# mila-iqia/babyai

Hardware: AMD Instinct MI355X
Metric: env-steps/sec (higher is better)
Workload: dtype u8; 1 GPU; BabyAI-BossLevel-v0 56x56x3 pixel (RGBImgPartialObsWrapper) obs, 1048576 envs in total = 1048576 per GPU x 1, random actions, auto-reset; envs_per_gpu=1048576, total_envs=1048576, parallelism=env-shards x1, no collective

## Files before the change

babyai_amd/csrc/bbai_render.hpp:

```cpp
#pragma once
#include "bbai_types.hpp"

namespace bbai {

constexpr int RENDER_QUEUE_DEFAULT = 1;
constexpr int RENDER_QUEUE_PACED = 3;
constexpr int64_t RENDER_QUEUE_MIN_ENVS = 262144;

constexpr int CHUNKS_PER_ROW = PIX * 3 / 8;
constexpr int VEC_PER_ENV = PIX_BYTES / 16;

constexpr int LINE_BYTES = 128;
constexpr int DELTA_UNIT = 8;
constexpr int UNIT_LINES = DELTA_UNIT * PIX_BYTES / LINE_BYTES;
static_assert(DELTA_UNIT * PIX_BYTES % LINE_BYTES == 0 && PIX_BYTES % 64 == 0, "8-env units are whole 128-byte lines");
constexpr int RENDER_PIECE_DEFAULT = 64;

BB_HD uint64_t line_cells(int s, int t) {
    uint64_t m = 0;
    for (int b = s; b < t; b += 8) {
        const int ch = b >> 3, py = ch / CHUNKS_PER_ROW, cx = ch - py * CHUNKS_PER_ROW;
        m |= 1ull << ((cx / 3) * VIEW + (py >> 3));
    }
    return m;
}

BB_HD constexpr uint32_t chunk_half_recipe(int byte) {
    const int row = byte / (PIX * 3), xb = byte - row * (PIX * 3);
    const int cell = xb / (TILE * 3) * VIEW + row / TILE;
    const int off = row % TILE * (TILE * 3) + xb % (TILE * 3);
    return (uint32_t)cell | (uint32_t)off << 8;
}
BB_HD constexpr uint32_t chunk_recipe(int k) { return chunk_half_recipe(16 * k) | chunk_half_recipe(16 * k + 8) << 16; }

BB_HD constexpr bool chunk_recipes_match_render_chunk() {
    for (int k = 0; k < VEC_PER_ENV; ++k) {
        uint32_t w = 0;
        for (int h = 0; h < 2; ++h) {
            const int ch = 2 * k + h;
            const int py = ch / CHUNKS_PER_ROW, cx = ch - py * CHUNKS_PER_ROW;
            const int ti = cx / 3, part = cx - ti * 3;
            const int tj = py >> 3, ty = py & 7;
            const int cell = ti * VIEW + tj, off = ty * 24 + part * 8;
            if (cell < 0 || cell >= VIEW * VIEW || off < 0 || off + 8 > TILE_BYTES) return false;
            w |= ((uint32_t)cell | (uint32_t)off << 8) << (16 * h);
        }
        if (chunk_recipe(k) != w) return false;
    }
    return true;
}
static_assert(TILE == 8 && TILE_BYTES <= 256 && VIEW * VIEW <= 256, "a cell and a tile offset fit a byte each");
static_assert(chunk_recipes_match_render_chunk(), "chunk_recipe(k) = render_chunk's (cell, offset) of chunks 2k and 2k + 1, for every k");

template <int P>
struct Pieces {
    static_assert(P == 16 || P == 32 || P == 64, "pieces of 16, 32 or 64 bytes");
    static_assert(PIX_BYTES % P == 0, "whole pieces per env");
    static constexpr int NP = PIX_BYTES / P;
    static constexpr int S = P / 16;
};

}

#if defined(__HIPCC__)
#include "bbai_kernels.hpp"

using namespace bbai;

__device__ __forceinline__ void load_atlas_lds(uint8_t* s_atlas, const uint8_t* atlas, int n_tiles, int tid, int T) {
    for (int k = tid; k < n_tiles * TILE_BYTES / 8; k += T) ((uint64_t*)s_atlas)[k] = ((const uint64_t*)atlas)[k];
}
__device__ __forceinline__ void load_lut_lds(uint8_t* s_lut, const uint8_t* lut, int tid, int T) {
    for (int k = tid; k < 512; k += T) s_lut[k] = lut[k];
}

__device__ __forceinline__ uint8_t tile_id(const uint8_t* s_lut, int o0, int o1, int o2, int cell) {
    const int key = o0 | (o1 << 3) | (o2 << 6);
    return s_lut[(cell == AGENT_CELL ? 256 : 0) + key];
}

__device__ __forceinline__ uint64_t render_chunk(const uint8_t* s_atlas, const uint8_t* tiles49, int ch) {
    const int py = ch / CHUNKS_PER_ROW, cx = ch - py * CHUNKS_PER_ROW;
    const int ti = cx / 3, part = cx - ti * 3;
    const int tj = py >> 3, ty = py & 7;
    const int tile = tiles49[ti * VIEW + tj];
    return *(const uint64_t*)(s_atlas + tile * TILE_BYTES + ty * 24 + part * 8);
}

__device__ __forceinline__ void store_chunk16(const uint8_t* s_atlas, const uint8_t* t49, int k, u32x4* dst) {
    const uint64_t lo = render_chunk(s_atlas, t49, 2 * k);
    const uint64_t hi = render_chunk(s_atlas, t49, 2 * k + 1);
    u32x4 v = {(uint32_t)lo, (uint32_t)(lo >> 32), (uint32_t)hi, (uint32_t)(hi >> 32)};
    __builtin_nontemporal_store(v, dst);
}

__device__ __forceinline__ void init_chunk_table(uint32_t* s_ct, int tid, int T) {
    for (int k = tid; k < bbai::VEC_PER_ENV; k += T) s_ct[k] = bbai::chunk_recipe(k);
}
__device__ __forceinline__ void store_chunk16_t(const uint8_t* s_atlas, const uint32_t* s_ct, const uint8_t* t49, int k, u32x4* dst) {
    const uint32_t w = s_ct[k];
    const uint32_t ta = t49[w & 0xff], tb = t49[(w >> 16) & 0xff];
    const uint64_t lo = *(const uint64_t*)(s_atlas + ta * TILE_BYTES + ((w >> 8) & 0xff));
    const uint64_t hi = *(const uint64_t*)(s_atlas + tb * TILE_BYTES + (w >> 24));
    u32x4 v = {(uint32_t)lo, (uint32_t)(lo >> 32), (uint32_t)hi, (uint32_t)(hi >> 32)};
    __builtin_nontemporal_store(v, dst);
}

template <int RENDER_GROUP, int RENDER_BLOCK>
__global__ __launch_bounds__(RENDER_BLOCK) void k_render(int64_t n, const uint8_t* __restrict__ image,
                                                         uint8_t* __restrict__ pixels, const uint8_t* __restrict__ atlas,
                                                         const uint8_t* __restrict__ lut, int n_tiles,
                                                         uint8_t* __restrict__ shadow ) {
    __shared__ __attribute__((aligned(16))) uint8_t s_atlas[MAX_TILES * TILE_BYTES];
    __shared__ uint8_t s_lut[512];
    __shared__ uint8_t s_tile[RENDER_GROUP * VIEW * VIEW + 8];
    load_atlas_lds(s_atlas, atlas, n_tiles, threadIdx.x, RENDER_BLOCK);
    load_lut_lds(s_lut, lut, threadIdx.x, RENDER_BLOCK);
    const int64_t ngroups = (n + RENDER_GROUP - 1) / RENDER_GROUP;
    for (int64_t grp = blockIdx.x; grp < ngroups; grp += gridDim.x) {
        const int64_t env0 = grp * RENDER_GROUP;
        const int ne = (int)(n - env0 < RENDER_GROUP ? n - env0 : RENDER_GROUP);
        __syncthreads();
        for (int c = threadIdx.x; c < ne * VIEW * VIEW; c += RENDER_BLOCK) {
            const int e = c / (VIEW * VIEW), cell = c - e * (VIEW * VIEW);
            const uint8_t* o = image + (env0 + e) * OBS_BYTES + cell * 3;
            s_tile[c] = tile_id(s_lut, o[0], o[1], o[2], cell);
            if (shadow) shadow[env0 * (VIEW * VIEW) + c] = s_tile[c];
        }
        __syncthreads();
        u32x4* out = (u32x4*)(pixels + env0 * PIX_BYTES);
        for (int q = threadIdx.x; q < ne * VEC_PER_ENV; q += RENDER_BLOCK) {
            const int e = q / VEC_PER_ENV, k = q - e * VEC_PER_ENV;
            store_chunk16(s_atlas, s_tile + e * (VIEW * VIEW), k, out + q);
        }
    }
}

template <int RENDER_GROUP, int RENDER_BLOCK, int NC, int K>
__global__ __launch_bounds__(RENDER_BLOCK) void k_render_q(int64_t n, const uint8_t* __restrict__ image,
                                                           uint8_t* __restrict__ pixels, const uint8_t* __restrict__ atlas,
                                                           const uint8_t* __restrict__ lut, int n_tiles, unsigned int* __restrict__ counters,
                                                           int pace_x16 ,
                                                           uint8_t* __restrict__ shadow ) {
    __shared__ __attribute__((aligned(16))) uint8_t s_atlas[MAX_TILES * TILE_BYTES];
    __shared__ uint8_t s_lut[512];
    __shared__ uint8_t s_tile[2][RENDER_GROUP * VIEW * VIEW + 8];
    __shared__ unsigned int s_ticket[2];
    __shared__ unsigned long long s_origin;
    load_atlas_lds(s_atlas, atlas, n_tiles, threadIdx.x, RENDER_BLOCK);
    load_lut_lds(s_lut, lut, threadIdx.x, RENDER_BLOCK);
    const int64_t all_groups = (n + RENDER_GROUP - 1) / RENDER_GROUP;
    const int64_t n_super = (all_groups + K - 1) / K;
    const unsigned int cidx = blockIdx.x % NC;
    unsigned int* counter = counters + 64 * cidx;
    int buf = 0, tp = 0;
    if (threadIdx.x == 0) {
        const unsigned int t0 = atomicAdd(counter, 1u);
        s_ticket[0] = t0;
        s_origin = __builtin_amdgcn_s_memrealtime() * 160ull - ((unsigned long long)t0 * NC + cidx) * (unsigned long long)pace_x16;
    }
    __syncthreads();
    for (;;) {
        const int64_t sg = (int64_t)s_ticket[tp] * NC + cidx;
        if (sg >= n_super) break;
        if (pace_x16) {
            const unsigned long long due = s_origin + (unsigned long long)sg * (unsigned long long)pace_x16;
            while (__builtin_amdgcn_s_memrealtime() * 160ull < due) __builtin_amdgcn_s_sleep(1);
        }
#pragma unroll
        for (int kk = 0; kk < K; ++kk) {
            const int64_t grp = sg * K + kk;
            if (grp >= all_groups) break;
            const int64_t env0 = grp * RENDER_GROUP;
            const int ne = (int)(n - env0 < RENDER_GROUP ? n - env0 : RENDER_GROUP);
            for (int c = threadIdx.x; c < ne * VIEW * VIEW; c += RENDER_BLOCK) {
                const int e = c / (VIEW * VIEW), cell = c - e * (VIEW * VIEW);
                const uint8_t* o = image + (env0 + e) * OBS_BYTES + cell * 3;
                s_tile[buf][c] = tile_id(s_lut, o[0], o[1], o[2], cell);
                if (shadow) shadow[env0 * (VIEW * VIEW) + c] = s_tile[buf][c];
            }
            if (kk == 0 && threadIdx.x == 0) s_ticket[tp ^ 1] = atomicAdd(counter, 1u);
            __syncthreads();
            u32x4* out = (u32x4*)(pixels + env0 * PIX_BYTES);
            for (int q = threadIdx.x; q < ne * VEC_PER_ENV; q += RENDER_BLOCK) {
                const int e = q / VEC_PER_ENV, k = q - e * VEC_PER_ENV;
                store_chunk16(s_atlas, s_tile[buf] + e * (VIEW * VIEW), k, out + q);
            }
            buf ^= 1;
        }
        tp ^= 1;
    }
    if (threadIdx.x == 0) {
        unsigned int* departed = counters + 64 * NC;
        if (atomicAdd(departed, 1u) == gridDim.x - 1) {
            for (int c = 0; c <= NC; ++c) atomicExch(counters + 64 * c, 0u);
        }
    }
}


__device__ __forceinline__ uint64_t delta_cell(const uint8_t* s_lut, uint32_t o0, uint32_t o1, uint32_t o2, uint32_t old, bool live, int lane,
                                               uint8_t* t49, uint8_t* shadow_row) {
    const uint32_t id = live ? tile_id(s_lut, o0, o1, o2, lane) : 0;
    const bool d = live && id != old;
    const uint64_t m = __ballot(d);
    if (live) t49[lane] = (uint8_t)id;
    if (d) shadow_row[lane] = (uint8_t)id;
    return m;
}

__device__ __forceinline__ void init_line_table(uint8_t* s_lea, uint64_t* s_lma, uint64_t* s_lmb, int tid, int T) {
    for (int l = tid; l < UNIT_LINES; l += T) {
        const int b0 = l * LINE_BYTES, b1 = b0 + LINE_BYTES;
        const int ea = b0 / PIX_BYTES, eb = (b1 - 1) / PIX_BYTES;
        s_lea[l] = (uint8_t)ea;
        s_lma[l] = line_cells(b0 - ea * PIX_BYTES, (eb != ea ? (ea + 1) * PIX_BYTES : b1) - ea * PIX_BYTES);
        s_lmb[l] = eb != ea ? line_cells(0, b1 - eb * PIX_BYTES) : 0;
    }
}

__device__ __forceinline__ void list_dirty_lines(const uint64_t* dmask, const uint8_t* s_lea, const uint64_t* s_lma, const uint64_t* s_lmb,
                                                 uint16_t* list, unsigned int* nd, int nl, int tid, int T) {
    const int lane = tid & 63;
    for (int L0 = tid - lane; L0 < nl; L0 += T) {
        const int L = L0 + lane;
        bool d = false;
        if (L < nl) {
            const int u = L / UNIT_LINES, l = L - u * UNIT_LINES, ea = u * DELTA_UNIT + s_lea[l];
            d = ((dmask[ea] & s_lma[l]) | (s_lmb[l] ? dmask[ea + 1] & s_lmb[l] : 0)) != 0;
        }
        const uint64_t m = __ballot(d);
        if (!m) continue;
        unsigned int base = 0;
        if (lane == 0) base = atomicAdd(nd, (unsigned int)__builtin_popcountll(m));
        base = __shfl(base, 0);
        if (d) list[base + __builtin_popcountll(m & ((1ull << lane) - 1))] = (uint16_t)L;
    }
}

__device__ __forceinline__ void store_listed_lines(const uint16_t* list, int nd, const uint8_t* s_atlas, const uint8_t* tiles, u32x4* out, int nq,
                                                   int tid, int T) {
    for (int i = tid; i < nd * 8; i += T) {
        const int q = (int)list[i >> 3] * 8 + (i & 7);
        if (q >= nq) continue;
        const int e = q / VEC_PER_ENV, k = q - e * VEC_PER_ENV;
        store_chunk16(s_atlas, tiles + e * CELLS, k, out + q);
    }
}

__device__ __forceinline__ void wave_lds_sync() {
    __builtin_amdgcn_fence(__ATOMIC_RELEASE, "workgroup");
    __builtin_amdgcn_wave_barrier();
    __builtin_amdgcn_fence(__ATOMIC_ACQUIRE, "workgroup");
}

template <int P>
__device__ __forceinline__ void init_piece_cells(uint64_t* s_pm, int tid, int nthreads) {
    for (int p = tid; p < Pieces<P>::NP; p += nthreads) s_pm[p] = line_cells(p * P, p * P + P);
}

template <int P>
__device__ __forceinline__ void store_dirty_pieces(uint64_t m, const uint64_t* s_pm, uint16_t* wl, const uint8_t* s_atlas, const uint32_t* s_ct,
                                                   const uint8_t* t49, u32x4* out, int lane) {
    constexpr int NP = Pieces<P>::NP, S = Pieces<P>::S;
    int cnt = 0;
    for (int p0 = 0; p0 < NP; p0 += 64) {
        const int p = p0 + lane;
        const bool d = p < NP && (m & s_pm[p]) != 0;
        const uint64_t b = __ballot(d);
        if (d) wl[cnt + __builtin_popcountll(b & ((1ull << lane) - 1))] = (uint16_t)p;
        cnt += __builtin_popcountll(b);
    }
    wave_lds_sync();
    for (int i = lane; i < cnt * S; i += 64) {
        const int k = (int)wl[i / S] * S + (i & (S - 1));
        store_chunk16_t(s_atlas, s_ct, t49, k, out + k);
    }
    wave_lds_sync();
}

template <int G, int T, int SCHED, int P>
__global__ __launch_bounds__(T) void k_render_delta(int64_t n, const uint8_t* __restrict__ image, uint8_t* __restrict__ pixels,
                                                    uint8_t* __restrict__ shadow ,
                                                    const uint8_t* __restrict__ atlas, const uint8_t* __restrict__ lut, int n_tiles) {
    static_assert(G % DELTA_UNIT == 0 && T % 64 == 0 && G % (T / 64) == 0, "whole units per group, whole envs per wave");
    constexpr int W = T / 64, EPW = G / W, GL = G / DELTA_UNIT * UNIT_LINES;
    __shared__ __attribute__((aligned(16))) uint8_t s_atlas[MAX_TILES * TILE_BYTES];
    __shared__ uint8_t s_lut[512];
    const int lane = threadIdx.x & 63, wave = threadIdx.x >> 6;
    const int64_t ngroups = (n + G - 1) / G;
    int64_t g, gend, gstep;
    if (SCHED == 0) { g = blockIdx.x; gend = ngroups; gstep = gridDim.x; }
    else { const int64_t per = (ngroups + gridDim.x - 1) / gridDim.x; g = blockIdx.x * per; gend = g + per < ngroups ? g + per : ngroups; gstep = 1; }
    uint32_t o0[EPW], o1[EPW], o2[EPW], old[EPW];
    auto load = [&](int64_t grp) {
#pragma unroll
        for (int j = 0; j < EPW; ++j) {
            const int64_t env = grp * G + wave + j * W;
            o0[j] = o1[j] = o2[j] = old[j] = 0;
            if (grp < gend && lane < CELLS && env < n) {
                const uint8_t* o = image + env * OBS_BYTES + lane * 3;
                o0[j] = o[0]; o1[j] = o[1]; o2[j] = o[2];
                old[j] = shadow[env * CELLS + lane];
            }
        }
    };
    load_atlas_lds(s_atlas, atlas, n_tiles, threadIdx.x, T);
    load_lut_lds(s_lut, lut, threadIdx.x, T);
    if constexpr (P < LINE_BYTES) {
        __shared__ uint64_t s_pm[Pieces<P>::NP];
        __shared__ uint16_t s_wl[W][Pieces<P>::NP];
        __shared__ uint8_t s_tile1[G * CELLS + 8];
        __shared__ uint32_t s_ct[VEC_PER_ENV];
        init_piece_cells<P>(s_pm, threadIdx.x, T);
        init_chunk_table(s_ct, threadIdx.x, T);
        load(g);
        __syncthreads();
        for (; g < gend; g += gstep) {
            const int64_t env0 = g * G;
            const int ne = (int)(n - env0 < G ? n - env0 : G);
            uint64_t dm[EPW];
#pragma unroll
            for (int j = 0; j < EPW; ++j) {
                const int e = wave + j * W;
                const bool live = lane < CELLS && e < ne;
                const uint32_t id = live ? tile_id(s_lut, o0[j], o1[j], o2[j], lane) : 0;
                const bool d = live && id != old[j];
                dm[j] = __ballot(d);
                if (live) s_tile1[e * CELLS + lane] = (uint8_t)id;
                if (d) shadow[(env0 + e) * CELLS + lane] = (uint8_t)id;
            }
            load(g + gstep);
            wave_lds_sync();
#pragma unroll
            for (int j = 0; j < EPW; ++j) {
                const int e = wave + j * W;
                if (dm[j]) store_dirty_pieces<P>(dm[j], s_pm, s_wl[wave], s_atlas, s_ct, s_tile1 + e * CELLS, (u32x4*)(pixels + (env0 + e) * PIX_BYTES), lane);
            }
        }
        return;
    } else {
    __shared__ uint64_t s_lma[UNIT_LINES], s_lmb[UNIT_LINES];
    __shared__ uint8_t s_lea[UNIT_LINES];
    __shared__ uint64_t s_dmask[2][G];
    __shared__ uint8_t s_tile[2][G * CELLS + 8];
    __shared__ uint16_t s_list[2][GL];
    __shared__ unsigned int s_nd[2];
    init_line_table(s_lea, s_lma, s_lmb, threadIdx.x, T);
    load(g);
    __syncthreads();
    int buf = 0;
    for (; g < gend; g += gstep, buf ^= 1) {
        const int64_t env0 = g * G;
        const int ne = (int)(n - env0 < G ? n - env0 : G);
#pragma unroll
        for (int j = 0; j < EPW; ++j) {
            const int e = wave + j * W;
            const uint64_t m = delta_cell(s_lut, o0[j], o1[j], o2[j], old[j], lane < CELLS && e < ne, lane, s_tile[buf] + e * CELLS, shadow + (env0 + e) * CELLS);
            if (lane == 0) s_dmask[buf][e] = m;
        }
        if (threadIdx.x == 0) s_nd[buf] = 0;
        __syncthreads();
        const int nl = (int)(((int64_t)ne * PIX_BYTES + LINE_BYTES - 1) / LINE_BYTES);
        list_dirty_lines(s_dmask[buf], s_lea, s_lma, s_lmb, s_list[buf], &s_nd[buf], nl, threadIdx.x, T);
        __syncthreads();
        const int64_t gn = g + gstep;
        load(gn);
        store_listed_lines(s_list[buf], (int)s_nd[buf], s_atlas, s_tile[buf], (u32x4*)(pixels + env0 * PIX_BYTES), ne * VEC_PER_ENV, threadIdx.x, T);
    }
    }
}

constexpr int DSTORE_PIECES = 32 * CELLS / 8;
template <int G, int T, int P>
__global__ __launch_bounds__(T) void k_render_dstore(int64_t n, uint8_t* __restrict__ pixels, const uint8_t* __restrict__ shadow ,
                                                     const uint64_t* __restrict__ dmask , const uint8_t* __restrict__ atlas, int n_tiles) {
    static_assert(G == 32 && T >= DSTORE_PIECES && T >= G && T % 64 == 0, "one 8-byte shadow piece per thread and group");
    constexpr int GL = G / DELTA_UNIT * UNIT_LINES;
    __shared__ __attribute__((aligned(16))) uint8_t s_atlas[MAX_TILES * TILE_BYTES];
    __shared__ __attribute__((aligned(8))) uint8_t s_tile[2][G * CELLS + 8];
    load_atlas_lds(s_atlas, atlas, n_tiles, threadIdx.x, T);
    const int tid = threadIdx.x, lane = tid & 63;
    const int64_t ngroups = (n + G - 1) / G;
    const int64_t gstep = gridDim.x;
    int64_t g = blockIdx.x;
    auto load_mask = [&](int64_t grp) -> uint64_t {
        const int64_t env = grp * G + tid;
        return (tid < G && grp < ngroups && env < n) ? dmask[env] : 0ull;
    };
    auto load_piece = [&](int64_t grp) -> uint2 {
        const int64_t base = grp * G * CELLS + 8 * tid, end = n * CELLS;
        if (base + 8 <= end) return *(const uint2*)(shadow + base);
        uint32_t w[2] = {0u, 0u};
        for (int i = 0; i < 8 && base + i < end; ++i) w[i >> 2] |= (uint32_t)shadow[base + i] << (8 * (i & 3));
        return make_uint2(w[0], w[1]);
    };
    if constexpr (P < LINE_BYTES) {
        constexpr int W = T / 64, EPW = G / W;
        __shared__ uint64_t s_pm[Pieces<P>::NP];
        __shared__ uint16_t s_wl[W][Pieces<P>::NP];
        __shared__ uint64_t s_dm3[3][G];
        __shared__ uint32_t s_ct[VEC_PER_ENV];
        const int wave = tid >> 6;
        init_piece_cells<P>(s_pm, tid, T);
        init_chunk_table(s_ct, tid, T);
        auto load_ids = [&](int64_t grp, int b) -> uint2 {
            if (tid >= DSTORE_PIECES || grp >= ngroups) return make_uint2(0u, 0u);
            const int ea = (8 * tid) / CELLS, eb = (8 * tid + 7) / CELLS;
            if (!s_dm3[b][ea] && !s_dm3[b][eb]) return make_uint2(0u, 0u);
            return load_piece(grp);
        };
        if (tid < G) s_dm3[0][tid] = load_mask(g);
        uint64_t mreg = load_mask(g + gstep);
        __syncthreads();
        uint2 idr = load_ids(g, 0);
        int buf = 0, mb = 0;
        for (; g < ngroups; g += gstep, buf ^= 1, mb = mb == 2 ? 0 : mb + 1) {
            const int64_t env0 = g * G;
            const int mn = mb == 2 ? 0 : mb + 1;
            if (tid < DSTORE_PIECES) *(uint2*)(s_tile[buf] + 8 * tid) = idr;
            if (tid < G) s_dm3[mn][tid] = mreg;
            __syncthreads();
            idr = load_ids(g + gstep, mn);
            mreg = load_mask(g + 2 * gstep);
#pragma unroll
            for (int j = 0; j < EPW; ++j) {
                const int e = wave + j * W;
                const uint64_t m = s_dm3[mb][e];
                if (m) store_dirty_pieces<P>(m, s_pm, s_wl[wave], s_atlas, s_ct, s_tile[buf] + e * CELLS, (u32x4*)(pixels + (env0 + e) * PIX_BYTES), lane);
            }
        }
        return;
    } else {
    __shared__ uint64_t s_lma[UNIT_LINES], s_lmb[UNIT_LINES];
    __shared__ uint8_t s_lea[UNIT_LINES];
    __shared__ uint64_t s_dmask[2][G];
    __shared__ uint16_t s_list[2][GL];
    __shared__ unsigned int s_nd[2];
    init_line_table(s_lea, s_lma, s_lmb, tid, T);
    const uint64_t shared_a = line_cells(PIX_BYTES - LINE_BYTES / 2, PIX_BYTES), shared_b = line_cells(0, LINE_BYTES / 2);
    static_assert(PIX_BYTES % LINE_BYTES == LINE_BYTES / 2, "two envs of a pair share one line");
    auto drawn = [&](int b, int e, int c0, int c1) -> bool {
        if (s_dmask[b][e]) return true;
        const uint64_t pm = (c1 == 63 ? ~0ull : (2ull << c1) - 1) & ~((1ull << c0) - 1);
        const bool shared_stored = ((s_dmask[b][e & ~1] & shared_a) | (s_dmask[b][e | 1] & shared_b)) != 0;
        return shared_stored && (pm & ((e & 1) ? shared_b : shared_a)) != 0;
    };
    auto load_ids = [&](int64_t grp, int b) -> uint2 {
        uint2 r = make_uint2(0u, 0u);
        if (tid >= DSTORE_PIECES || grp >= ngroups) return r;
        const int b0 = 8 * tid, b1 = b0 + 7, ea = b0 / CELLS, eb = b1 / CELLS;
        const bool need = eb == ea ? drawn(b, ea, b0 - ea * CELLS, b1 - ea * CELLS) : (drawn(b, ea, b0 - ea * CELLS, CELLS - 1) || drawn(b, eb, 0, b1 - eb * CELLS));
        if (!need) return r;
        return load_piece(grp);
    };
    if (tid < G) s_dmask[0][tid] = load_mask(g);
    uint64_t mreg = load_mask(g + gstep);
    __syncthreads();
    uint2 idr = load_ids(g, 0);
    int buf = 0;
    for (; g < ngroups; g += gstep, buf ^= 1) {
        const int64_t env0 = g * G;
        const int ne = (int)(n - env0 < G ? n - env0 : G);
        if (tid < DSTORE_PIECES) *(uint2*)(s_tile[buf] + 8 * tid) = idr;
        if (tid < G) s_dmask[buf ^ 1][tid] = mreg;
        if (tid == 0) s_nd[buf] = 0;
        __syncthreads();
        const int nl = (int)(((int64_t)ne * PIX_BYTES + LINE_BYTES - 1) / LINE_BYTES);
        for (int L0 = tid - lane; L0 < nl; L0 += T) {
            const int L = L0 + lane;
            bool d = false;
            if (L < nl) {
                const int u = L / UNIT_LINES, l = L - u * UNIT_LINES, ea = u * DELTA_UNIT + s_lea[l];
                d = ((s_dmask[buf][ea] & s_lma[l]) | (s_lmb[l] ? s_dmask[buf][ea + 1] & s_lmb[l] : 0)) != 0;
            }
            const uint64_t m = __ballot(d);
            if (!m) continue;
            unsigned int base = 0;
            if (lane == 0) base = atomicAdd(&s_nd[buf], (unsigned int)__builtin_popcountll(m));
            base = __shfl(base, 0);
            if (d) s_list[buf][base + __builtin_popcountll(m & ((1ull << lane) - 1))] = (uint16_t)L;
        }
        idr = load_ids(g + gstep, buf ^ 1);
        mreg = load_mask(g + 2 * gstep);
        __syncthreads();
        store_listed_lines(s_list[buf], (int)s_nd[buf], s_atlas, s_tile[buf], (u32x4*)(pixels + env0 * PIX_BYTES), ne * VEC_PER_ENV, tid, T);
    }
    }
}

constexpr int DSTORE_LW_T = 9 * 64;
constexpr int DSTORE_LW_K = 2;
constexpr int DSTORE_LW_COUNTER = 32 * 64, DSTORE_LW_DEPARTED = 33 * 64;
__device__ __forceinline__ int64_t uniform64(int64_t v) {
    return (int64_t)(((uint64_t)(uint32_t)__builtin_amdgcn_readfirstlane((int)((uint64_t)v >> 32)) << 32) | (uint32_t)__builtin_amdgcn_readfirstlane((int)v));
}
template <int P>
__global__ __launch_bounds__(DSTORE_LW_T) void k_render_dstore_lw(int64_t n, uint8_t* __restrict__ pixels, const uint8_t* __restrict__ shadow ,
                                                                  const uint64_t* __restrict__ dmask , const uint8_t* __restrict__ atlas, int n_tiles,
                                                                  unsigned int* __restrict__ tickets) {
    static_assert(P < LINE_BYTES, "pieces");
    constexpr int G = 32, T = DSTORE_LW_T, W = 8, K = DSTORE_LW_K, ROUNDS = (DSTORE_PIECES + 63) / 64;
    __shared__ __attribute__((aligned(16))) uint8_t s_atlas[MAX_TILES * TILE_BYTES];
    __shared__ __attribute__((aligned(8))) uint8_t s_tile[2][G * CELLS + 8];
    __shared__ uint64_t s_pm[Pieces<P>::NP];
    __shared__ uint16_t s_wl[W][Pieces<P>::NP];
    __shared__ uint64_t s_dm3[3][G];
    __shared__ uint32_t s_ct[VEC_PER_ENV];
    __shared__ uint8_t s_list[3][G];
    __shared__ unsigned int s_cnt[3], s_next[3];
    __shared__ int64_t s_grp[3];
    __shared__ unsigned int s_spare;
    const int tid = threadIdx.x, lane = tid & 63;
    const int wave = __builtin_amdgcn_readfirstlane(tid >> 6);
    const bool loader = wave == W;
    const int64_t ngroups = (n + G - 1) / G;
    load_atlas_lds(s_atlas, atlas, n_tiles, tid, T);
    init_piece_cells<P>(s_pm, tid, T);
    init_chunk_table(s_ct, tid, T);
    unsigned int* counter = tickets + DSTORE_LW_COUNTER;
    int64_t g1 = ngroups;
    auto loader_step = [&](int k, int m1, int tb, int m2) {
        const int64_t end = n * CELLS;
        const bool opens = (k + 2) % K == 0;
        int64_t g2 = g1 + 1;
        unsigned int spare = 0;
        if (opens) {
            g2 = (int64_t)s_spare * K;
            if (lane == 0) spare = atomicAdd(counter, 1u);
        }
        uint2 v[ROUNDS];
        bool need[ROUNDS], tail = false;
#pragma unroll
        for (int r = 0; r < ROUNDS; ++r) {
            const int p = r * 64 + lane, pc = p < DSTORE_PIECES ? p : DSTORE_PIECES - 1;
            const int64_t base = g1 * G * CELLS + 8 * p;
            need[r] = p < DSTORE_PIECES && g1 < ngroups && (s_dm3[m1][(8 * pc) / CELLS] || s_dm3[m1][(8 * pc + 7) / CELLS]);
            const bool whole = base + 8 <= end;
            tail |= need[r] && !whole;
            v[r] = *(const uint2*)(shadow + (need[r] && whole ? base : 0));
        }
        const int64_t env = g2 * G + lane;
        const bool live = lane < G && g2 < ngroups && env < n;
        uint64_t m = dmask[live ? env : 0];
        if (!live) m = 0;
        if (__any(tail)) {
#pragma unroll
            for (int r = 0; r < ROUNDS; ++r) {
                const int64_t base = g1 * G * CELLS + 8 * (r * 64 + lane);
                if (!need[r] || base + 8 <= end) continue;
                uint32_t w[2] = {0u, 0u};
                for (int i = 0; i < 8 && base + i < end; ++i) w[i >> 2] |= (uint32_t)shadow[base + i] << (8 * (i & 3));
                v[r] = make_uint2(w[0], w[1]);
            }
        }
#pragma unroll
        for (int r = 0; r < ROUNDS; ++r) {
            const int p = r * 64 + lane;
            if (p < DSTORE_PIECES) *(uint2*)(s_tile[tb] + 8 * p) = need[r] ? v[r] : make_uint2(0u, 0u);
        }
        if (lane < G) s_dm3[m2][lane] = m;
        const uint64_t dirty = __ballot(m != 0);
        if (m) s_list[m2][__builtin_popcountll(dirty & ((1ull << lane) - 1))] = (uint8_t)lane;
        if (lane == 0) {
            s_cnt[m2] = (unsigned int)__builtin_popcountll(dirty);
            s_next[m2] = 0;
            s_grp[m2] = g2;
            if (opens) s_spare = spare;
        }
        g1 = g2;
    };
    if (loader) {
        if (lane == 0) s_spare = atomicAdd(counter, 1u);
        wave_lds_sync();
        loader_step(-2, 2, 1, 0);
        wave_lds_sync();
        loader_step(-1, 0, 0, 1);
    }
    __syncthreads();
    int buf = 0, mb = 0;
    for (int k = 0;; ++k, buf ^= 1, mb = mb == 2 ? 0 : mb + 1) {
        const int64_t g = uniform64(s_grp[mb]);
        if (g >= ngroups) break;
        if (loader) {
            const int m1 = mb == 2 ? 0 : mb + 1, m2 = m1 == 2 ? 0 : m1 + 1;
            loader_step(k, m1, buf ^ 1, m2);
        } else {
            const int64_t env0 = g * G;
            const unsigned int cnt = __builtin_amdgcn_readfirstlane(s_cnt[mb]);
            for (;;) {
                unsigned int i = 0;
                if (lane == 0) i = atomicAdd(&s_next[mb], 1u);
                i = __builtin_amdgcn_readfirstlane(i);
                if (i >= cnt) break;
                const int e = __builtin_amdgcn_readfirstlane(s_list[mb][i]);
                store_dirty_pieces<P>(s_dm3[mb][e], s_pm, s_wl[wave], s_atlas, s_ct, s_tile[buf] + e * CELLS, (u32x4*)(pixels + (env0 + e) * PIX_BYTES), lane);
            }
        }
        __syncthreads();
    }
    if (tid == W * 64) {
        unsigned int* departed = tickets + DSTORE_LW_DEPARTED;
        if (atomicAdd(departed, 1u) == gridDim.x - 1) { atomicExch(counter, 0u); atomicExch(departed, 0u); }
    }
}
#endif
```

Baseline: 1.768 billion env-steps/s.

## Replace dynamic dirty-piece worklist with static per-lane chunk mapping in dstore kernel

The dirty-store kernel no longer builds a per-wave LDS worklist of dirty 64-byte pieces through ballots. Each lane instead owns a fixed set of 16-byte chunks whose cell recipes and cell masks are computed at compile time and held in registers. All tile-id and atlas reads are issued before the stores, and the next env index and mask are prefetched from LDS while the current env's reads are in flight. This removes the s_pm, s_wl and s_ct tables and their wave syncs. In exchange, lanes with clean chunks sit idle, register pressure rises, and the kernel is restricted to 64-byte pieces.

```diff
diff --git a/babyai_amd/csrc/bbai_render.hpp b/babyai_amd/csrc/bbai_render.hpp
--- a/babyai_amd/csrc/bbai_render.hpp
+++ b/babyai_amd/csrc/bbai_render.hpp
@@ -16,7 +16,7 @@
 static_assert(DELTA_UNIT * PIX_BYTES % LINE_BYTES == 0 && PIX_BYTES % 64 == 0, "8-env units are whole 128-byte lines");
 constexpr int RENDER_PIECE_DEFAULT = 64;
 
-BB_HD uint64_t line_cells(int s, int t) {
+BB_HD constexpr uint64_t line_cells(int s, int t) {
     uint64_t m = 0;
     for (int b = s; b < t; b += 8) {
         const int ch = b >> 3, py = ch / CHUNKS_PER_ROW, cx = ch - py * CHUNKS_PER_ROW;
@@ -59,6 +59,39 @@
     static constexpr int NP = PIX_BYTES / P;
     static constexpr int S = P / 16;
 };
+
+constexpr int STATIC_ROUNDS = (VEC_PER_ENV + 63) / 64;
+BB_HD constexpr int static_chunk(int r, int lane) { return 64 * r + lane; }
+BB_HD constexpr uint64_t static_chunk_cells(int r, int lane) {
+    const int k = static_chunk(r, lane);
+    return k < VEC_PER_ENV ? line_cells((k >> 2) * 64, (k >> 2) * 64 + 64) : 0;
+}
+BB_HD constexpr uint32_t static_chunk_recipe(int r, int lane) {
+    const int k = static_chunk(r, lane);
+    return k < VEC_PER_ENV ? chunk_recipe(k) : 0u;
+}
+BB_HD constexpr uint64_t round_cells(int r) {
+    uint64_t m = 0;
+    for (int p = 16 * r; p < 16 * r + 16 && p < Pieces<64>::NP; ++p) m |= line_cells(64 * p, 64 * p + 64);
+    return m;
+}
+BB_HD constexpr bool static_chunk_stored(uint64_t m, int r, int lane) {
+    return (m & round_cells(r)) != 0 && (m & static_chunk_cells(r, lane)) != 0;
+}
+BB_HD constexpr bool round_cells_match_line_cells() {
+    for (int r = 0; r < STATIC_ROUNDS; ++r) {
+        uint64_t m = 0;
+        for (int lane = 0; lane < 64; ++lane) {
+            const int k = static_chunk(r, lane);
+            if ((k < VEC_PER_ENV) != (static_chunk_cells(r, lane) != 0)) return false;
+            if (k < VEC_PER_ENV && static_chunk_cells(r, lane) != line_cells(k / 4 * 64, k / 4 * 64 + 64)) return false;
+            m |= static_chunk_cells(r, lane);
+        }
+        if (m != round_cells(r)) return false;
+    }
+    return STATIC_ROUNDS * 64 >= VEC_PER_ENV && (STATIC_ROUNDS - 1) * 64 < VEC_PER_ENV && VEC_PER_ENV - (STATIC_ROUNDS - 1) * 64 == 12;
+}
+static_assert(round_cells_match_line_cells(), "round_cells(r) = the OR of line_cells over the pieces of round r's live lanes; round 9 has 12 of them");
 
 }
 
@@ -277,6 +310,52 @@
         store_chunk16_t(s_atlas, s_ct, t49, k, out + k);
     }
     wave_lds_sync();
+}
+
+struct StaticLane { uint32_t recipe[STATIC_ROUNDS]; uint64_t cells[STATIC_ROUNDS]; };
+__device__ __forceinline__ void init_static_lane(StaticLane& sl, int lane) {
+#pragma unroll
+    for (int r = 0; r < STATIC_ROUNDS; ++r) { sl.recipe[r] = static_chunk_recipe(r, lane); sl.cells[r] = static_chunk_cells(r, lane); }
+}
+__device__ __forceinline__ void wait_lds_reads() { __builtin_amdgcn_s_waitcnt(0xc07f); }
+template <class F1, class F2>
+__device__ __forceinline__ void store_static_rounds(uint64_t m, const StaticLane& sl, const uint8_t* s_atlas, const uint8_t* t49, u32x4* out, int lane,
+                                                    F1 with_atlas, F2 with_stores) {
+    constexpr int R0 = 0, R1 = STATIC_ROUNDS;
+    uint32_t ta[R1 - R0], tb[R1 - R0];
+    uint64_t lo[R1 - R0], hi[R1 - R0];
+#pragma unroll
+    for (int r = R0; r < R1; ++r) {
+        const uint32_t w = sl.recipe[r];
+        ta[r - R0] = tb[r - R0] = 0;
+        if (m & round_cells(r)) {
+            if (m & sl.cells[r]) { ta[r - R0] = t49[w & 0xff]; tb[r - R0] = t49[(w >> 16) & 0xff]; }
+        }
+    }
+    wait_lds_reads();
+#pragma unroll
+    for (int r = R0; r < R1; ++r) {
+        const uint32_t w = sl.recipe[r];
+        lo[r - R0] = hi[r - R0] = 0;
+        if (m & round_cells(r)) {
+            if (m & sl.cells[r]) {
+                lo[r - R0] = *(const uint64_t*)(s_atlas + ta[r - R0] * TILE_BYTES + ((w >> 8) & 0xff));
+                hi[r - R0] = *(const uint64_t*)(s_atlas + tb[r - R0] * TILE_BYTES + (w >> 24));
+            }
+        }
+    }
+    with_atlas();
+    wait_lds_reads();
+    with_stores();
+#pragma unroll
+    for (int r = R0; r < R1; ++r) {
+        if (m & round_cells(r)) {
+            if (m & sl.cells[r]) {
+                u32x4 v = {(uint32_t)lo[r - R0], (uint32_t)(lo[r - R0] >> 32), (uint32_t)hi[r - R0], (uint32_t)(hi[r - R0] >> 32)};
+                __builtin_nontemporal_store(v, out + static_chunk(r, lane));
+            }
+        }
+    }
 }
 
 template <int G, int T, int SCHED, int P>
@@ -499,14 +578,11 @@
 __global__ __launch_bounds__(DSTORE_LW_T) void k_render_dstore_lw(int64_t n, uint8_t* __restrict__ pixels, const uint8_t* __restrict__ shadow ,
                                                                   const uint64_t* __restrict__ dmask , const uint8_t* __restrict__ atlas, int n_tiles,
                                                                   unsigned int* __restrict__ tickets) {
-    static_assert(P < LINE_BYTES, "pieces");
+    static_assert(P == 64, "the static lane-to-chunk mapping is that of 64-byte pieces");
     constexpr int G = 32, T = DSTORE_LW_T, W = 8, K = DSTORE_LW_K, ROUNDS = (DSTORE_PIECES + 63) / 64;
     __shared__ __attribute__((aligned(16))) uint8_t s_atlas[MAX_TILES * TILE_BYTES];
     __shared__ __attribute__((aligned(8))) uint8_t s_tile[2][G * CELLS + 8];
-    __shared__ uint64_t s_pm[Pieces<P>::NP];
-    __shared__ uint16_t s_wl[W][Pieces<P>::NP];
     __shared__ uint64_t s_dm3[3][G];
-    __shared__ uint32_t s_ct[VEC_PER_ENV];
     __shared__ uint8_t s_list[3][G];
     __shared__ unsigned int s_cnt[3], s_next[3];
     __shared__ int64_t s_grp[3];
@@ -516,8 +592,6 @@
     const bool loader = wave == W;
     const int64_t ngroups = (n + G - 1) / G;
     load_atlas_lds(s_atlas, atlas, n_tiles, tid, T);
-    init_piece_cells<P>(s_pm, tid, T);
-    init_chunk_table(s_ct, tid, T);
     unsigned int* counter = tickets + DSTORE_LW_COUNTER;
     int64_t g1 = ngroups;
     auto loader_step = [&](int k, int m1, int tb, int m2) {
@@ -570,12 +644,15 @@
         }
         g1 = g2;
     };
+    StaticLane sl = {};
     if (loader) {
         if (lane == 0) s_spare = atomicAdd(counter, 1u);
         wave_lds_sync();
         loader_step(-2, 2, 1, 0);
         wave_lds_sync();
         loader_step(-1, 0, 0, 1);
+    } else {
+        init_static_lane(sl, lane);
     }
     __syncthreads();
     int buf = 0, mb = 0;
@@ -588,13 +665,28 @@
         } else {
             const int64_t env0 = g * G;
             const unsigned int cnt = __builtin_amdgcn_readfirstlane(s_cnt[mb]);
-            for (;;) {
-                unsigned int i = 0;
-                if (lane == 0) i = atomicAdd(&s_next[mb], 1u);
-                i = __builtin_amdgcn_readfirstlane(i);
-                if (i >= cnt) break;
-                const int e = __builtin_amdgcn_readfirstlane(s_list[mb][i]);
-                store_dirty_pieces<P>(s_dm3[mb][e], s_pm, s_wl[wave], s_atlas, s_ct, s_tile[buf] + e * CELLS, (u32x4*)(pixels + (env0 + e) * PIX_BYTES), lane);
+            unsigned int* const take = &s_next[mb] + ((tid >> 6) - wave);
+            unsigned int iv = 0;
+            if (lane == 0) iv = atomicAdd(take, 1u);
+            unsigned int i = __builtin_amdgcn_readfirstlane(iv);
+            int e = 0;
+            uint64_t m = 0;
+            if (i < cnt) {
+                e = __builtin_amdgcn_readfirstlane(s_list[mb][i]);
+                m = (uint64_t)uniform64((int64_t)s_dm3[mb][e]);
+            }
+            while (i < cnt) {
+                unsigned int nv = 0, ev = 0;
+                uint64_t mv = 0;
+                if (lane == 0) nv = atomicAdd(take, 1u);
+                const uint8_t* t49 = s_tile[buf] + e * CELLS;
+                u32x4* out = (u32x4*)(pixels + (env0 + e) * PIX_BYTES);
+                store_static_rounds(m, sl, s_atlas, t49, out, lane,
+                                    [&] { if (lane == 0) ev = s_list[mb][nv < cnt ? nv : 0u]; },
+                                    [&] { if (lane == 0) mv = s_dm3[mb][ev & (G - 1)]; });
+                i = __builtin_amdgcn_readfirstlane(nv);
+                e = __builtin_amdgcn_readfirstlane(ev) & (G - 1);
+                m = (uint64_t)uniform64((int64_t)mv);
             }
         }
         __syncthreads();
```

Result: slower. 1.748 billion env-steps/s (-1.1%).
